# douban/dpark

Measured on NVIDIA H100. Metric: shuffled rows/sec (reduceByKey end-to-end), higher is better.
Workload: dtype int64

## Files before the change

__graft_entry__.py:

```python
import os
import subprocess
import sys

ROOT = os.path.dirname(os.path.abspath(__file__))
if ROOT not in sys.path:
    sys.path.insert(0, ROOT)


def build():
    subprocess.check_call(["make", "-s", "-j8", "-C", os.path.join(ROOT, "dpark_b200", "csrc")])
    subprocess.check_call(["make", "-s", "-C", os.path.join(ROOT, "oracle"), "all"])
    from oracle import build_reference
    if os.path.exists(os.path.join(build_reference.REF, "dpark", "portable_hash.pyx")):
        subprocess.call(["make", "-s", "-C", os.path.join(ROOT, "oracle"), "ref", "REF=" + build_reference.REF])
        subprocess.call([sys.executable, os.path.join(ROOT, "oracle", "build_reference.py")])
    subprocess.check_call(
        ["nvcc", "-gencode", "arch=compute_90a,code=sm_90a", "-O2", "-std=c++17", "-Xcompiler", "-fPIC",
         "-shared", "-I" + os.path.join(ROOT, "include"), "-I" + os.path.join(ROOT, "dpark_b200", "csrc"),
         os.path.join(ROOT, "tests", "hostcheck.cu"), os.path.join(ROOT, "dpark_b200", "csrc", "dpk_core.o"),
         "-o", os.path.join(ROOT, "tests", "_hostcheck.so")])
    import dpark_b200
    from dpark_b200 import _native
    _native.lib()


def smoke():
    import numpy as np
    import torch
    from dpark_b200 import _native as nv
    from dpark_b200 import shuffle
    from oracle import oracle as orc

    assert torch.cuda.is_available(), "smoke() needs cuda:0"
    torch.cuda.set_device(0)
    rng = np.random.default_rng(0)
    n, P, M = 200000, 8, 4
    k = rng.integers(-5000, 5000, n, dtype=np.int64)
    v = rng.integers(0, 1 << 16, n, dtype=np.int64)
    ks, vs = np.array_split(k, M), np.array_split(v, M)
    before = nv.launch_count()
    res = shuffle.reduce_by_key([torch.from_numpy(x).cuda() for x in ks],
                                [torch.from_numpy(x).cuda() for x in vs], P, "sum")
    torch.cuda.synchronize()
    assert nv.launch_count() > before, "no CUDA kernels were launched"
    want = orc.reduce_by_key(ks, vs, P, "sum")
    for p, gk, gv in res:
        gk, gv = gk.cpu().numpy(), gv.cpu().numpy()
        wk, wv = want[p]
        o1, o2 = np.argsort(gk), np.argsort(wk)
        assert np.array_equal(gk[o1], wk[o2]) and np.array_equal(gv[o1], wv[o2]), "partition %d differs" % p
    print("smoke ok: reduceByKey over %d rows, %d partitions, %d kernel launches, matches oracle"
          % (n, P, nv.launch_count() - before))


if __name__ == "__main__":
    build()
    if len(sys.argv) > 1 and sys.argv[1] == "smoke":
        smoke()
```

dpark_b200/csrc/dpk_common.cuh:

```cuda
#pragma once
#include <cuda_runtime.h>
#include <stdint.h>
#include <stdio.h>
#include <stdarg.h>
#include <string.h>
#include <math.h>

#include "dpark_b200.h"

#define DPK_HD __host__ __device__ __forceinline__

namespace dpk {

extern thread_local char g_err[512];
int fail(int code, const char *fmt, ...);
#define DPK_CUDA_TRY(expr)                                                        \
    do {                                                                          \
        cudaError_t _e = (expr);                                                  \
        if (_e != cudaSuccess)                                                    \
            return dpk::fail(DPK_ERR_CUDA, "%s failed: %s (%s:%d)", #expr,        \
                             cudaGetErrorString(_e), __FILE__, __LINE__);         \
    } while (0)
#define DPK_LAUNCH_CHECK() DPK_CUDA_TRY(cudaGetLastError())

// ... 110 lines not shown
struct PartFn {
    int32_t P;
    int32_t mode;
    uint64_t magic;
    int32_t shift;
    int32_t nthr;
    const int64_t *thresholds;
    int32_t sub_bits;
    const int64_t *row_hash;

    DPK_HD int32_t nbuckets() const { return P << sub_bits; }
    DPK_HD int32_t bucket(int64_t h) const {
        if (mode == 4) return (int32_t)(((uint64_t)h >> shift) & (uint64_t)(P - 1));
        if (mode == 5) return P == 1 ? 0 : (int32_t)((mixed(h) >> shift) & (uint32_t)(P - 1));
        int32_t p = (*this)(h);
        if (sub_bits == 0) return p;
        return (p << sub_bits) | (int32_t)(mixed(h) >> (32 - sub_bits));
    }
    static DPK_HD uint32_t mixed(int64_t h) {
        uint32_t x = (uint32_t)(uint64_t)h * 0x9E3779B1u + (uint32_t)((uint64_t)h >> 32) * 0x85EBCA77u;
        x ^= x >> 16; x *= 0x21F0AAADu;
        x ^= x >> 15; x *= 0x735A2D97u;
        x ^= x >> 15;
        return x;
    }

    DPK_HD int32_t operator()(int64_t h) const {
        if (mode == 1) return (int32_t)((uint64_t)h & (uint64_t)(P - 1));
        if (mode == 2) {
            uint64_t a = h < 0 ? 0ull - (uint64_t)h : (uint64_t)h;
#ifdef __CUDA_ARCH__
            uint64_t q = __umul64hi(magic, a);
#else
            uint64_t q = (uint64_t)(((unsigned __int128)magic * a) >> 64);
#endif
            uint64_t t = ((a - q) >> 1) + q;
            q = t >> shift;
            uint32_t r = (uint32_t)(a - q * (uint64_t)P);
            return h < 0 ? (r ? P - (int32_t)r : 0) : (int32_t)r;
        }
        if (mode == 3) {
            int32_t lo = 0, hi = nthr;
            while (lo < hi) {
                int32_t mid = (lo + hi) >> 1;
                if (h < thresholds[mid]) hi = mid; else lo = mid + 1;
            }
            return lo;
        }
        return 0;
    }
};
int make_partfn(int32_t P, const int64_t *thresholds, int32_t nthr, int32_t sub_bits, PartFn *out);

int64_t seg_multisplit_ws_bytes(int64_t n, int32_t F1, int32_t S2, int32_t nsrc);
int seg_multisplit(const void *keys, int key_kind, const void *vals, int32_t val_bytes, int64_t n,
                   const PartFn &fine, int32_t F1, int32_t nsrc, const int64_t *seg_start,
                   const int64_t *seg_rows, void *out_keys, void *out_vals, int64_t *fine_off, void *ws,
                   int64_t ws_bytes, cudaStream_t st, bool stable = false);

DPK_HD uint64_t mix64(uint64_t x) {
    x ^= x >> 33; x *= 0xff51afd7ed558ccdull; x ^= x >> 33; x *= 0xc4ceb9fe1a85ec53ull;
    return x ^ (x >> 33);
}
DPK_HD uint32_t slot_hash32(uint64_t kb) {
    uint32_t x = (uint32_t)kb * 0xCC9E2D51u + (uint32_t)(kb >> 32) * 0x1B873593u + 0x7F4A7C15u;
    x ^= x >> 16; x *= 0x85EBCA6Bu;
    x ^= x >> 13; x *= 0xC2B2AE35u;
    x ^= x >> 16;
    return x;
}

constexpr int AG_MAX_SB2 = 10;
DPK_HD int choose_sb2(int64_t n, int32_t F, int target_rows) {
    int sb2 = 0;
    while (sb2 < AG_MAX_SB2 && n / ((int64_t)F << sb2) > target_rows) sb2++;
    return sb2;
}
DPK_HD PartFn fine_partfn(const PartFn &first, int sb2) {
    PartFn fine = first;
    fine.mode = 5; fine.P = 1 << sb2; fine.shift = 32 - first.sub_bits - sb2; fine.sub_bits = 0;
    return fine;
}

constexpr int TK_BYTES = 16;
__host__ __device__ __forceinline__ bool tok_ws(uint8_t c) { return c == 0x20 || (c >= 0x09 && c <= 0x0d) || (c >= 0x1c && c <= 0x1f); }

__host__ __device__ __forceinline__ uint32_t tok_starts16(const uint8_t *__restrict__ data, int64_t n, int64_t i0, bool *hi) {
    uint8_t c[TK_BYTES];
    if (i0 + TK_BYTES <= n && (((uintptr_t)(data + i0)) & 15u) == 0) {
        const uint4 q = *reinterpret_cast<const uint4 *>(data + i0);
        const uint32_t w[4] = {q.x, q.y, q.z, q.w};
#pragma unroll
        for (int j = 0; j < TK_BYTES; j++) c[j] = (uint8_t)(w[j >> 2] >> ((j & 3) * 8));
    } else {
#pragma unroll
        for (int j = 0; j < TK_BYTES; j++) c[j] = i0 + j < n ? data[i0 + j] : (uint8_t)0x20;
    }
    bool prev_ws = i0 == 0 ? true : tok_ws(data[i0 - 1]);
    uint32_t m = 0;
    bool h = false;
#pragma unroll
    for (int j = 0; j < TK_BYTES; j++) {
        const bool ws = tok_ws(c[j]);
        h |= c[j] >= 0x80;
        if (!ws && prev_ws) m |= 1u << j;
        prev_ws = ws;
    }
    *hi = h;
    return m;
}


}
```

dpark_b200/csrc/dpk_partition.cu:

```cuda
#include "dpk_common.cuh"

namespace dpk {

constexpr int PT_THREADS = 256;
constexpr int PT_WARPS = PT_THREADS / 32;
constexpr int PT_ITEMS = 16;
constexpr int PT_TILE = PT_THREADS * PT_ITEMS;
constexpr int PT_COUNT_PRIV = 1024;

struct NoVal {};

int g_count_mode = 1;
int g_scatter_items = 16;
int g_scatter_bulk = 1;
int g_scatter_threads = 512;
int g_scatter_seg_wide = 1;
int g_scatter_wide_from = 512;
int g_scatter_ptr_bulk = 1;
int g_scatter_ptr_threads = 1024;

struct SegTab {
    const int64_t *cbeg, *cend;
    const int32_t *ctotal;
    int32_t *chunk_counts;
    const int64_t *chunk_off;
    const uint64_t *key_ptrs, *val_ptrs;
    int unordered;
};

struct Plan {
    int32_t T;
    int64_t L;
    SegTab seg;
    const char *label_count = nullptr, *label_scatter = nullptr;
};

static Plan make_plan(int64_t n) {
    Plan pl;
    pl.seg = SegTab{nullptr, nullptr, nullptr, nullptr, nullptr, nullptr, nullptr, 0};
    int64_t tiles = (n + PT_TILE - 1) / PT_TILE;
    if (tiles < 1) tiles = 1;
    int64_t maxT = (int64_t)sm_count() * 8;
    pl.T = (int32_t)(tiles < maxT ? tiles : maxT);
    pl.L = tiles;
    return pl;
}

static inline int64_t align_up(int64_t x, int64_t a) { return (x + a - 1) / a * a; }

static int64_t ws_counts_bytes(int32_t P) { return align_up((int64_t)P * sm_count() * 8 * 4, 256); }
static int64_t ws_total_bytes(int32_t P) {
    return ws_counts_bytes(P) + align_up((int64_t)P * 8, 256) + align_up((int64_t)(P + 1) * 8, 256);
}

template <typename KeyT, int PRE>
__device__ __forceinline__ int64_t key_hash(KeyT k, const PartFn &f) {
    if constexpr (PRE == 1) return (int64_t)k;
    else if constexpr (PRE == 2) return __ldg(&f.row_hash[(int64_t)k]);
    else return KeyHash<KeyT>::of(k);
}

__device__ __forceinline__ unsigned warp_peers(int id, int nbits) {
    unsigned peers = 0xffffffffu;
#pragma unroll
    for (int b = 0; b < 13; b++) {
        if (b < nbits) {
            const unsigned set = __ballot_sync(0xffffffffu, (id >> b) & 1);
            peers &= ((id >> b) & 1) ? set : ~set;
        }
    }
    return peers;
}

template <int NW = PT_WARPS>
__device__ __forceinline__ int block_excl_scan(int v, int *s_warp, int *total) {
    const int lane = threadIdx.x & 31, warp = threadIdx.x >> 5;
    int inc = v;
#pragma unroll
    for (int d = 1; d < 32; d <<= 1) {
        int t = __shfl_up_sync(0xffffffffu, inc, d);
        if (lane >= d) inc += t;
    }
    if (lane == 31) s_warp[warp] = inc;
    __syncthreads();
    int base = 0, tot = 0;
#pragma unroll
    for (int w = 0; w < NW; w++) {
        int t = s_warp[w];
        if (w < warp) base += t;
        tot += t;
    }
    __syncthreads();
    *total = tot;
    return base + inc - v;
}

template <typename KeyT, int PRE>
__global__ void __launch_bounds__(PT_THREADS)
k_part_count(const KeyT *__restrict__ keys, int64_t n, int64_t L, PartFn f,
             int32_t *__restrict__ tile_counts, int32_t T, SegTab seg, int count_mode) {
    extern __shared__ int32_t s_cnt[];
    const int P = f.nbuckets();
    if (seg.cbeg != nullptr && (int)blockIdx.x >= *seg.ctotal) return;
    const bool priv = P <= PT_COUNT_PRIV;
    const int nhist = priv ? PT_WARPS * P : P;
    for (int p = threadIdx.x; p < nhist; p += PT_THREADS) s_cnt[p] = 0;
    __syncthreads();
    const int64_t beg = seg.cbeg ? seg.cbeg[blockIdx.x] : ((int64_t)blockIdx.x * L / T) * PT_TILE;
    const int64_t end = seg.cbeg ? seg.cend[blockIdx.x] : min(n, ((int64_t)(blockIdx.x + 1) * L / T) * PT_TILE);
    const int lane = threadIdx.x & 31;
    int32_t *wh = s_cnt + (priv ? (threadIdx.x >> 5) * P : 0);
    constexpr int U = 8;
    int64_t i0 = beg;
    if (count_mode == 1) {
        for (; i0 + (int64_t)PT_THREADS * U <= end; i0 += (int64_t)PT_THREADS * U) {
            KeyT k[U];
#pragma unroll
            for (int u = 0; u < U; u++) k[u] = keys[i0 + (int64_t)u * PT_THREADS + threadIdx.x];
#pragma unroll
            for (int u = 0; u < U; u++) atomicAdd(&wh[f.bucket(key_hash<KeyT, PRE>(k[u], f))], 1);
        }
    }
    for (; i0 < end; i0 += (int64_t)PT_THREADS * U) {
        KeyT k[U];
        bool ok[U];
#pragma unroll
        for (int u = 0; u < U; u++) {
            int64_t i = i0 + (int64_t)u * PT_THREADS + threadIdx.x;
            ok[u] = i < end;
            k[u] = ok[u] ? keys[i] : KeyT(0);
        }
// ... 359 lines not shown
                const int p = bucket_of<FMODE>(f, key_hash<KeyT, PRE>(k[j], f));
                pr[j] = ((uint32_t)p << 16) | atomicAdd(&cnt[p], 1u);
            }
        } else {
            const int left = (int)(end - tile) - warp * (32 * ITEMS) - lane;
#pragma unroll
            for (int j = 0; j < ITEMS; j++) {
                pr[j] = 0xffffffffu;
                if (j * 32 < left) {
                    const int p = bucket_of<FMODE>(f, key_hash<KeyT, PRE>(k[j], f));
                    pr[j] = ((uint32_t)p << 16) | atomicAdd(&cnt[p], 1u);
                }
            }
        }
        asm volatile("cp.async.bulk.wait_group.read 0;" ::: "memory");
        __syncthreads();

        {
            const int b = threadIdx.x * E;
            int sum = 0;
            for (int i = b; i < min(b + E, P); i++) sum += (int)cnt[i];
            int tot;
            int run = block_excl_scan<NW>(sum, s_warp, &tot);
            for (int i = b; i < min(b + E, P); i++) {
                const int64_t g = s_gpos[i];
                const uint32_t gk = (uint32_t)(((uintptr_t)(out_keys + g)) / sizeof(KeyT));
                const int basek = run + i * (AK - 1);
                s_sk[i] = basek + (int)((gk - (uint32_t)basek) & (uint32_t)(AK - 1));
                if constexpr (HAS_VAL) {
                    const uint32_t gv = (uint32_t)(((uintptr_t)(out_vals + (ptrs ? g + s_vd[i] : g))) / sizeof(ValT));
                    const int basev = run + i * (AV - 1);
                    s_sv[i] = basev + (int)((gv - (uint32_t)basev) & (uint32_t)(AV - 1));
                }
                run += (int)cnt[i];
            }
        }
        __syncthreads();

#pragma unroll
        for (int j = 0; j < ITEMS; j++) {
            const int p = (int)(pr[j] >> 16), r = (int)(pr[j] & 0xffffu);
            if (p != 0xffff) {
                s_key[s_sk[p] + r] = k[j];
                if constexpr (HAS_VAL) s_val[s_sv[p] + r] = v[j];
            }
        }
        if (tile + TILE < end) load_tile(tile + TILE);
        asm volatile("fence.proxy.async.shared::cta;" ::: "memory");
        __syncthreads();

        if constexpr (HAS_VAL) {
            for (int q0 = 0; q0 < 2 * P; q0 += NT) {
                const int q = q0 + (int)threadIdx.x;
                const int p = q >> 1;
                const bool on = q < 2 * P;
                const int c = on ? (int)cnt[p] : 0;
                const int64_t g = on ? s_gpos[p] : 0;
                if (c) {
                    if (q & 1) flush_run<ValT>(out_vals, ptrs ? g + s_vd[p] : g, s_val, val_addr, s_sv[p], c);
                    else flush_run<KeyT>(out_keys, g, s_key, key_addr, s_sk[p], c);
                }
                __syncwarp();
                if (c && !(q & 1)) {
                    s_gpos[p] = g + c;
                    cnt[p] = 0;
                }
            }
        } else {
            for (int p = threadIdx.x; p < P; p += NT) {
                const int c = (int)cnt[p];
                if (c) {
                    const int64_t g = s_gpos[p];
                    flush_run<KeyT>(out_keys, g, s_key, key_addr, s_sk[p], c);
                    s_gpos[p] = g + c;
                    cnt[p] = 0;
                }
            }
        }
        asm volatile("cp.async.bulk.commit_group;" ::: "memory");
    }
    asm volatile("cp.async.bulk.wait_group 0;" ::: "memory");
}

template <typename KeyT, int PRE>
static int launch_count(const void *keys, int64_t n, const Plan &pl, const PartFn &f,
                        int32_t *tile_counts, cudaStream_t st) {
    size_t sh = (size_t)f.nbuckets() * sizeof(int32_t) * (f.nbuckets() <= PT_COUNT_PRIV ? PT_WARPS : 1);
    DPK_LAUNCH(pl.label_count ? pl.label_count : (pl.seg.cbeg ? "seg_count" : "part_count"), st, k_part_count<KeyT, PRE><<<pl.T, PT_THREADS, sh, st>>>((const KeyT *)keys, n, pl.L, f, tile_counts, pl.T, pl.seg, g_count_mode));
    return DPK_OK;
}

static int dispatch_count(const void *keys, int key_kind, int64_t n, const Plan &pl, const PartFn &f,
                          int32_t *tile_counts, cudaStream_t st) {
    if (key_kind >= DPK_K_UNORDERED) key_kind -= DPK_K_UNORDERED;
    switch (key_kind) {
    case -1: return launch_count<int64_t, true>(keys, n, pl, f, tile_counts, st);
    case DPK_K_I64: return launch_count<int64_t, false>(keys, n, pl, f, tile_counts, st);
    case DPK_K_I32: return launch_count<int32_t, false>(keys, n, pl, f, tile_counts, st);
    case DPK_K_F64: return launch_count<double, false>(keys, n, pl, f, tile_counts, st);
    case DPK_K_U64: return launch_count<uint64_t, false>(keys, n, pl, f, tile_counts, st);
    case DPK_K_F32: return launch_count<float, false>(keys, n, pl, f, tile_counts, st);
    case DPK_K_ROWID:
        if (!f.row_hash) return fail(DPK_ERR_INVALID, "DPK_K_ROWID needs key_aux (the per-row hash column)");
        return launch_count<int64_t, 2>(keys, n, pl, f, tile_counts, st);
    }
    return fail(DPK_ERR_UNSUPPORTED, "key kind %d is unhashable by portable_hash", key_kind);
}

template <typename KeyT, typename ValT, int PRE, int ITEMS>
static int launch_scatter_items(const void *keys, const void *vals, int64_t n, const Plan &pl, const PartFn &f,
                                const int32_t *tile_off, const int64_t *bucket_base, void *out_keys,
                                void *out_vals, cudaStream_t st) {
    constexpr int vb = std::is_same<ValT, NoVal>::value ? 0 : (int)sizeof(ValT);
    ScatterSmem lay = scatter_smem((int)sizeof(KeyT), vb, f.nbuckets(), pl.seg.key_ptrs != nullptr, PT_THREADS * ITEMS);
    auto kern = k_part_scatter<KeyT, ValT, PRE, ITEMS>;
    if (lay.total > 227 * 1024)
        return fail(DPK_ERR_UNSUPPORTED, "%d buckets need %lld B of shared memory", f.nbuckets(), (long long)lay.total);
    DPK_CUDA_TRY(cudaFuncSetAttribute(kern, cudaFuncAttributeMaxDynamicSharedMemorySize, (int)lay.total));
    DPK_LAUNCH(pl.label_scatter ? pl.label_scatter : (pl.seg.cbeg ? "seg_scatter" : "part_scatter"), st,
               kern<<<pl.T, PT_THREADS, (size_t)lay.total, st>>>((const KeyT *)keys, (const ValT *)vals, n, pl.L, f,
                                                                tile_off, pl.T, bucket_base, (KeyT *)out_keys,
                                                                (ValT *)out_vals, lay, pl.seg));
    return DPK_OK;
}

template <typename KeyT, typename ValT, int PRE>
static int launch_scatter_bulk(const void *keys, const void *vals, int64_t n, const Plan &pl, const PartFn &f,
                               const int32_t *tile_off, const int64_t *bucket_base, void *out_keys,
                               void *out_vals, cudaStream_t st) {
    constexpr int vb = std::is_same<ValT, NoVal>::value ? 0 : (int)sizeof(ValT);
    int nt = g_scatter_threads;
    if (nt == 512 && pl.seg.cbeg != nullptr && g_scatter_seg_wide) nt = 1024;
    if (nt == 512 && g_scatter_seg_wide && sizeof(KeyT) <= 4 && (vb == 0 || vb <= 4)) nt = 1024;
    if (nt == 512 && g_scatter_wide_from > 0 && f.nbuckets() >= g_scatter_wide_from) nt = 1024;
    const bool ptr_mode = pl.seg.key_ptrs != nullptr;
    if (ptr_mode && nt == 512 && g_scatter_ptr_threads == 1024) nt = 1024;
    if (nt == 1024 && bulk_smem((int)sizeof(KeyT), vb, f.nbuckets(), 8192, ptr_mode).total > 220 * 1024) nt = 512;
    BulkSmem lay = bulk_smem((int)sizeof(KeyT), vb, f.nbuckets(), nt == 1024 ? 8192 : PT_TILE, ptr_mode);
    const int fmode = f.mode == 5 ? 2 : ((f.mode == 0 || f.mode == 1) ? 1 : 0);
    if (ptr_mode) {
        auto kp = nt == 1024 ? (fmode == 1 ? k_part_scatter_bulk<KeyT, ValT, PRE, 1024, 1, true> : k_part_scatter_bulk<KeyT, ValT, PRE, 1024, 0, true>)
                             : (fmode == 1 ? k_part_scatter_bulk<KeyT, ValT, PRE, 512, 1, true> : k_part_scatter_bulk<KeyT, ValT, PRE, 512, 0, true>);
        if (nt != 512 && nt != 1024) return fail(DPK_ERR_UNSUPPORTED, "pointer mode needs 512- or 1024-thread CTAs");
        DPK_CUDA_TRY(cudaFuncSetAttribute(kp, cudaFuncAttributeMaxDynamicSharedMemorySize, (int)lay.total));
        DPK_LAUNCH(pl.label_scatter ? pl.label_scatter : "part_scatter", st,
                   kp<<<pl.T, nt, (size_t)lay.total, st>>>((const KeyT *)keys, (const ValT *)vals, n, pl.L, f, tile_off, pl.T,
                                                          bucket_base, (KeyT *)out_keys, (ValT *)out_vals, lay, pl.seg));
        return DPK_OK;
    }
    auto kern = nt == 1024 ? (fmode == 2 ? k_part_scatter_bulk<KeyT, ValT, PRE, 1024, 2> :
                              fmode == 1 ? k_part_scatter_bulk<KeyT, ValT, PRE, 1024, 1> : k_part_scatter_bulk<KeyT, ValT, PRE, 1024, 0>)
              : nt == 512 ? (fmode == 2 ? k_part_scatter_bulk<KeyT, ValT, PRE, 512, 2> :
                             fmode == 1 ? k_part_scatter_bulk<KeyT, ValT, PRE, 512, 1> : k_part_scatter_bulk<KeyT, ValT, PRE, 512, 0>)
                          : k_part_scatter_bulk<KeyT, ValT, PRE, 256, 0>;
    DPK_CUDA_TRY(cudaFuncSetAttribute(kern, cudaFuncAttributeMaxDynamicSharedMemorySize, (int)lay.total));
    DPK_LAUNCH(pl.label_scatter ? pl.label_scatter : (pl.seg.cbeg ? "seg_scatter" : "part_scatter"), st,
               kern<<<pl.T, nt, (size_t)lay.total, st>>>((const KeyT *)keys, (const ValT *)vals, n, pl.L, f,
                                                                tile_off, pl.T, bucket_base, (KeyT *)out_keys,
                                                                (ValT *)out_vals, lay, pl.seg));
    return DPK_OK;
}

template <typename KeyT, typename ValT, int PRE>
static int launch_scatter(const void *keys, const void *vals, int64_t n, const Plan &pl_in, const PartFn &f,
                          const int32_t *tile_off, const int64_t *bucket_base, void *out_keys,
                          void *out_vals, cudaStream_t st) {
    Plan pl = pl_in;
    if (pl.seg.unordered == 2) {
        constexpr int vb = std::is_same<ValT, NoVal>::value ? 0 : (int)sizeof(ValT);
        if (bulk_smem((int)sizeof(KeyT), vb, f.nbuckets(), PT_TILE, pl.seg.key_ptrs != nullptr).total <= 110 * 1024)
            return launch_scatter_bulk<KeyT, ValT, PRE>(keys, vals, n, pl, f, tile_off, bucket_base, out_keys, out_vals, st);
        pl.seg.unordered = (f.nbuckets() % 2 == 0) ? 1 : 0;
    }
    if (g_scatter_items == 8)
        return launch_scatter_items<KeyT, ValT, PRE, 8>(keys, vals, n, pl, f, tile_off, bucket_base, out_keys, out_vals, st);
    return launch_scatter_items<KeyT, ValT, PRE, 16>(keys, vals, n, pl, f, tile_off, bucket_base, out_keys, out_vals, st);
}

template <typename KeyT, int PRE>
static int dispatch_val(const void *keys, const void *vals, int32_t val_bytes, int64_t n, const Plan &pl,
                        const PartFn &f, const int32_t *tile_off, const int64_t *bucket_base,
                        void *out_keys, void *out_vals, cudaStream_t st) {
    if (vals == nullptr || val_bytes == 0)
        return launch_scatter<KeyT, NoVal, PRE>(keys, nullptr, n, pl, f, tile_off, bucket_base, out_keys, nullptr, st);
    if (val_bytes == 8)
        return launch_scatter<KeyT, int64_t, PRE>(keys, vals, n, pl, f, tile_off, bucket_base, out_keys, out_vals, st);
    if (val_bytes == 4)
        return launch_scatter<KeyT, int32_t, PRE>(keys, vals, n, pl, f, tile_off, bucket_base, out_keys, out_vals, st);
    return fail(DPK_ERR_UNSUPPORTED, "val_bytes must be 0, 4 or 8, got %d", val_bytes);
}

static int dispatch_scatter(const void *keys, int key_kind, const void *vals, int32_t val_bytes, int64_t n,
                            const Plan &pl_in, const PartFn &f, const int32_t *tile_off,
                            const int64_t *bucket_base, void *out_keys, void *out_vals, cudaStream_t st) {
    Plan pl = pl_in;
    if (key_kind >= DPK_K_UNORDERED) {
        key_kind -= DPK_K_UNORDERED;
        if (f.nbuckets() % 2 == 0) pl.seg.unordered = 1;
        if (g_scatter_bulk && (pl.seg.key_ptrs == nullptr || g_scatter_ptr_bulk)) pl.seg.unordered = 2;
    } else if (pl.seg.unordered && g_scatter_bulk && pl.seg.key_ptrs == nullptr) {
        pl.seg.unordered = 2;
    }
    switch (key_kind) {
    case -1: return dispatch_val<int64_t, true>(keys, vals, val_bytes, n, pl, f, tile_off, bucket_base, out_keys, out_vals, st);
    case DPK_K_I64: return dispatch_val<int64_t, false>(keys, vals, val_bytes, n, pl, f, tile_off, bucket_base, out_keys, out_vals, st);
    case DPK_K_I32: return dispatch_val<int32_t, false>(keys, vals, val_bytes, n, pl, f, tile_off, bucket_base, out_keys, out_vals, st);
    case DPK_K_F64: return dispatch_val<double, false>(keys, vals, val_bytes, n, pl, f, tile_off, bucket_base, out_keys, out_vals, st);
    case DPK_K_U64: return dispatch_val<uint64_t, false>(keys, vals, val_bytes, n, pl, f, tile_off, bucket_base, out_keys, out_vals, st);
    case DPK_K_F32: return dispatch_val<float, false>(keys, vals, val_bytes, n, pl, f, tile_off, bucket_base, out_keys, out_vals, st);
    case DPK_K_ROWID:
        if (!f.row_hash) return fail(DPK_ERR_INVALID, "DPK_K_ROWID needs key_aux (the per-row hash column)");
        return dispatch_val<int64_t, 2>(keys, vals, val_bytes, n, pl, f, tile_off, bucket_base, out_keys, out_vals, st);
    }
    return fail(DPK_ERR_UNSUPPORTED, "key kind %d is unhashable by portable_hash", key_kind);
}

static int check_common(const void *keys, int64_t n, int32_t P, int32_t sub_bits, void *ws, int64_t ws_bytes) {
    if (n < 0 || n >= ((int64_t)1 << 31)) return fail(DPK_ERR_INVALID, "n=%lld out of range [0, 2^31)", (long long)n);
    if (P < 1 || sub_bits < 0 || sub_bits > 12 || ((int64_t)P << sub_bits) > DPK_MAX_PARTITIONS)
        return fail(DPK_ERR_UNSUPPORTED, "P=%d (x 2^%d sub-buckets) out of range [1, %d]", P, sub_bits, DPK_MAX_PARTITIONS);
    P <<= sub_bits;
    if (n > 0 && !keys) return fail(DPK_ERR_INVALID, "keys is NULL");
// ... 68 lines not shown
        int t = s_tot[p];
        s_tot[p] = run;
        run += t;
    }
    __syncthreads();
    const int64_t base = brow_off[b];
    for (int p = threadIdx.x; p < S2; p += PT_THREADS) {
        int64_t pos = base + s_tot[p];
        fine_off[(int64_t)b * S2 + p] = pos;
        for (int64_t c = c0; c < c1; c++) {
            chunk_off[c * S2 + p] = pos;
            pos += chunk_counts[c * S2 + p];
        }
    }
    if (b == F1 - 1 && threadIdx.x == 0) fine_off[(int64_t)F1 * S2] = brow_off[F1];
}

int64_t seg_multisplit_ws_bytes(int64_t n, int32_t F1, int32_t S2, int32_t nsrc) {
    const int64_t maxc = seg_max_chunks(n, F1, nsrc);
    return align_up((int64_t)(F1 + 1) * 8, 256) * 2 + 256 + align_up(maxc * 8, 256) * 2 +
           align_up(maxc * S2 * 4, 256) + align_up(maxc * S2 * 8, 256);
}

int seg_multisplit(const void *keys, int key_kind, const void *vals, int32_t val_bytes, int64_t n,
                   const PartFn &fine, int32_t F1, int32_t nsrc, const int64_t *seg_start,
                   const int64_t *seg_rows, void *out_keys, void *out_vals, int64_t *fine_off, void *ws,
                   int64_t ws_bytes, cudaStream_t st, bool stable) {
    const int32_t S2 = fine.nbuckets();
    if (ws_bytes < seg_multisplit_ws_bytes(n, F1, S2, nsrc)) return fail(DPK_ERR_WORKSPACE, "segmented multisplit workspace too small");
    const int64_t maxc = seg_max_chunks(n, F1, nsrc);
    char *w = (char *)ws;
    int64_t *brow_off = (int64_t *)w; w += align_up((int64_t)(F1 + 1) * 8, 256);
    int64_t *cfirst = (int64_t *)w; w += align_up((int64_t)(F1 + 1) * 8, 256);
    int32_t *ctotal = (int32_t *)w; w += 256;
    int64_t *cbeg = (int64_t *)w; w += align_up(maxc * 8, 256);
    int64_t *cend = (int64_t *)w; w += align_up(maxc * 8, 256);
    int32_t *chunk_counts = (int32_t *)w; w += align_up(maxc * S2 * 4, 256);
    int64_t *chunk_off = (int64_t *)w;
    DPK_LAUNCH("seg_plan", st, k_seg_plan<<<1, PT_THREADS, 0, st>>>(seg_start, seg_rows, nsrc, F1, brow_off, cfirst, cbeg, cend, ctotal));
    Plan pl;
    pl.T = (int32_t)maxc;
    pl.L = 0;
    pl.seg = SegTab{cbeg, cend, ctotal, chunk_counts, chunk_off, nullptr, nullptr, (S2 % 2 == 0) ? 1 : (g_scatter_bulk ? 2 : 0)};
    if (stable) {
        pl.seg.unordered = 0;
        pl.label_count = "radix_count";
        pl.label_scatter = "radix_scatter";
    }
    int rc = DPK_OK;
    if (n > 0) {
        rc = dispatch_count(keys, key_kind, n, pl, fine, nullptr, st);
        if (rc) return rc;
    }
    DPK_LAUNCH("seg_scan", st, k_seg_scan<<<F1, PT_THREADS, (size_t)S2 * 4, st>>>(chunk_counts, cfirst, brow_off, F1, S2, chunk_off, fine_off));
    if (n > 0) rc = dispatch_scatter(keys, key_kind, vals, val_bytes, n, pl, fine, nullptr, nullptr, out_keys, out_vals, st);
    return rc;
}

}

using namespace dpk;

extern "C" {

int64_t dpk_partition_workspace_bytes(int64_t n, int32_t nbuckets) {
    (void)n;
    if (nbuckets < 1) nbuckets = 1;
    return ws_total_bytes(nbuckets);
}

int dpk_partition_count(const void *keys, int key_kind, const int64_t *key_aux, int64_t n, int32_t P,
                        const int64_t *thresholds, int32_t nthr, int32_t sub_bits, int64_t *out_counts,
                        void *ws, int64_t ws_bytes, dpk_stream_t stream) {
    int rc = check_common(keys, n, P, sub_bits, ws, ws_bytes);
    if (rc) return rc;
    if (!out_counts) return fail(DPK_ERR_INVALID, "out_counts is NULL");
    PartFn f;
    rc = make_partfn(P, thresholds, nthr, sub_bits, &f);
    if (rc) return rc;
    f.row_hash = key_aux;
    const int32_t F = f.nbuckets();
    cudaStream_t st = (cudaStream_t)stream;
    int32_t *tile_counts = (int32_t *)ws;
    Plan pl = make_plan(n);
    if (n == 0) {
        DPK_CUDA_TRY(cudaMemsetAsync(tile_counts, 0, (size_t)F * pl.T * 4, st));
    } else {
        rc = dispatch_count(keys, key_kind, n, pl, f, tile_counts, st);
        if (rc) return rc;
    }
    DPK_LAUNCH("part_scan", st, k_part_scan<<<F, PT_THREADS, 0, st>>>(tile_counts, pl.T, out_counts));
    return DPK_OK;
}

int dpk_partition_scatter(const void *keys, int key_kind, const int64_t *key_aux, const void *vals,
                          int32_t val_bytes, int64_t n, int32_t P, const int64_t *thresholds, int32_t nthr,
                          int32_t sub_bits,
                          const int64_t *bucket_base, void *out_keys, void *out_vals, void *ws,
                          int64_t ws_bytes, dpk_stream_t stream) {
    int rc = check_common(keys, n, P, sub_bits, ws, ws_bytes);
    if (rc) return rc;
    if (n == 0) return DPK_OK;
    if (!bucket_base || !out_keys) return fail(DPK_ERR_INVALID, "NULL pointer");
    PartFn f;
    rc = make_partfn(P, thresholds, nthr, sub_bits, &f);
    if (rc) return rc;
    f.row_hash = key_aux;
    Plan pl = make_plan(n);
    return dispatch_scatter(keys, key_kind, vals, val_bytes, n, pl, f, (const int32_t *)ws, bucket_base,
                            out_keys, out_vals, (cudaStream_t)stream);
}

int dpk_partition(const void *keys, int key_kind, const int64_t *key_aux, const void *vals, int32_t val_bytes,
                  int64_t n, int32_t P, const int64_t *thresholds, int32_t nthr, int32_t sub_bits, void *out_keys, void *out_vals,
                  int64_t *out_offsets, void *ws, int64_t ws_bytes, dpk_stream_t stream) {
    int rc = check_common(keys, n, P, sub_bits, ws, ws_bytes);
    if (rc) return rc;
    if (!out_offsets) return fail(DPK_ERR_INVALID, "out_offsets is NULL");
    const int32_t F = P << sub_bits;
    int64_t *totals = (int64_t *)((char *)ws + ws_counts_bytes(F));
    rc = dpk_partition_count(keys, key_kind, key_aux, n, P, thresholds, nthr, sub_bits, totals, ws, ws_bytes, stream);
    if (rc) return rc;
    cudaStream_t st = (cudaStream_t)stream;
    DPK_LAUNCH("part_offsets", st, k_part_offsets<<<1, PT_THREADS, 0, st>>>(totals, F, out_offsets));
    return dpk_partition_scatter(keys, key_kind, key_aux, vals, val_bytes, n, P, thresholds, nthr, sub_bits, out_offsets,
                                 out_keys, out_vals, ws, ws_bytes, stream);
}

int dpk_partition_scatter_ptrs(const void *keys, int key_kind, const int64_t *key_aux, const void *vals,
                               int32_t val_bytes, int64_t n, int32_t P, const int64_t *thresholds, int32_t nthr,
                               int32_t sub_bits, const uint64_t *key_dst_ptrs, const uint64_t *val_dst_ptrs,
                               void *ws, int64_t ws_bytes, dpk_stream_t stream) {
    int rc = check_common(keys, n, P, sub_bits, ws, ws_bytes);
    if (rc) return rc;
    if (n == 0) return DPK_OK;
    if (!key_dst_ptrs || (vals && val_bytes && !val_dst_ptrs)) return fail(DPK_ERR_INVALID, "NULL pointer table");
    PartFn f;
    rc = make_partfn(P, thresholds, nthr, sub_bits, &f);
    if (rc) return rc;
    f.row_hash = key_aux;
    Plan pl = make_plan(n);
    pl.seg.key_ptrs = key_dst_ptrs;
    pl.seg.val_ptrs = val_dst_ptrs;
    return dispatch_scatter(keys, key_kind, vals, val_bytes, n, pl, f, (const int32_t *)ws, nullptr, nullptr, nullptr,
                            (cudaStream_t)stream);
}

__global__ void __launch_bounds__(PT_THREADS)
k_seg_starts(const int64_t *__restrict__ seg_rows, int32_t nsrc, int32_t F, int64_t *__restrict__ seg_start) {
    __shared__ long long s_part[PT_THREADS];
    __shared__ long long s_carry;
    const int E = (F + PT_THREADS - 1) / PT_THREADS;
    const int b0 = threadIdx.x * E, b1 = min(b0 + E, F);
    if (threadIdx.x == 0) s_carry = 0;
    __syncthreads();
    for (int s = 0; s < nsrc; s++) {
        long long mine = 0;
        for (int b = b0; b < b1; b++) mine += seg_rows[(int64_t)s * F + b];
        s_part[threadIdx.x] = mine;
        __syncthreads();
        long long base = s_carry, tot = 0;
        for (int t = 0; t < PT_THREADS; t++) {
            if (t < (int)threadIdx.x) base += s_part[t];
            tot += s_part[t];
        }
        for (int b = b0; b < b1; b++) {
            seg_start[(int64_t)s * F + b] = base;
            base += seg_rows[(int64_t)s * F + b];
        }
        __syncthreads();
        if (threadIdx.x == 0) s_carry += tot;
        __syncthreads();
    }
}

int64_t dpk_radix_pass_seg_workspace_bytes(int64_t n, int32_t nbuckets, int32_t nsrc, int32_t bits) {
    if (n < 0) n = 0;
    if (nbuckets < 1) nbuckets = 1;
    if (nsrc < 1) nsrc = 1;
    return align_up((int64_t)nbuckets * nsrc * 8, 256) + seg_multisplit_ws_bytes(n, nbuckets, 1 << bits, nsrc);
}

int dpk_radix_pass_seg(const int64_t *keys, const void *vals, int32_t val_bytes, int64_t n, int32_t shift, int32_t bits,
                       int32_t nbuckets, int32_t nsrc, const int64_t *seg_rows, int64_t *out_keys, void *out_vals,
                       int64_t *out_fine_off, void *ws, int64_t ws_bytes, dpk_stream_t stream) {
    if (bits < 1 || bits > 10 || shift < 0 || shift > 63) return fail(DPK_ERR_INVALID, "bad radix digit shift=%d bits=%d", shift, bits);
    if (n < 0 || n >= ((int64_t)1 << 31)) return fail(DPK_ERR_INVALID, "n=%lld out of range [0, 2^31)", (long long)n);
    if (nbuckets < 1 || nsrc < 1 || !seg_rows || !out_fine_off || !ws) return fail(DPK_ERR_INVALID, "bad segment description");
    if (n > 0 && (!keys || !out_keys)) return fail(DPK_ERR_INVALID, "NULL pointer");
    if (ws_bytes < dpk_radix_pass_seg_workspace_bytes(n, nbuckets, nsrc, bits)) return fail(DPK_ERR_WORKSPACE, "workspace too small");
    cudaStream_t st = (cudaStream_t)stream;
    int64_t *seg_start = (int64_t *)ws;
    void *ws2 = (char *)ws + align_up((int64_t)nbuckets * nsrc * 8, 256);
    DPK_LAUNCH("seg_starts", st, k_seg_starts<<<1, PT_THREADS, 0, st>>>(seg_rows, nsrc, nbuckets, seg_start));
    PartFn f;
    f.P = 1 << bits; f.mode = 4; f.magic = 0; f.shift = shift; f.nthr = 0; f.thresholds = nullptr; f.sub_bits = 0;
    f.row_hash = nullptr;
    return seg_multisplit(keys, -1, vals, val_bytes, n, f, nbuckets, nsrc, seg_start, seg_rows, out_keys, out_vals,
                          out_fine_off, ws2, ws_bytes - align_up((int64_t)nbuckets * nsrc * 8, 256), st, true);
}

int dpk_radix_pass(const int64_t *keys, const void *vals, int32_t val_bytes, int64_t n, int32_t shift,
                   int32_t bits, int64_t *out_keys, void *out_vals, void *ws, int64_t ws_bytes,
                   dpk_stream_t stream) {
    if (bits < 1 || bits > 12 || shift < 0 || shift > 63)
        return fail(DPK_ERR_INVALID, "bad radix digit shift=%d bits=%d", shift, bits);
    const int32_t F = 1 << bits;
    int rc = check_common(keys, n, F, 0, ws, ws_bytes);
    if (rc) return rc;
    if (n == 0) return DPK_OK;
    if (!out_keys) return fail(DPK_ERR_INVALID, "NULL pointer");
    PartFn f;
    f.P = F; f.mode = 4; f.magic = 0; f.shift = shift; f.nthr = 0; f.thresholds = nullptr; f.sub_bits = 0;
    f.row_hash = nullptr;
    cudaStream_t st = (cudaStream_t)stream;
    int32_t *tile_counts = (int32_t *)ws;
    int64_t *totals = (int64_t *)((char *)ws + ws_counts_bytes(F));
    int64_t *offsets = (int64_t *)((char *)totals + align_up((int64_t)F * 8, 256));
    Plan pl = make_plan(n);
    pl.label_count = "radix_count";
    pl.label_scatter = "radix_scatter";
    rc = dispatch_count(keys, -1, n, pl, f, tile_counts, st);
    if (rc) return rc;
    DPK_LAUNCH("part_scan", st, k_part_scan<<<F, PT_THREADS, 0, st>>>(tile_counts, pl.T, totals));
// ... 6 lines not shown
```

Baseline: 15.42 billion.

## Add 2-CTA cluster scatter kernel sharing staging buffers via distributed shared memory

Adds a thread-block-cluster variant of the bulk partition scatter, used for unordered keys with many buckets. The two CTAs in a cluster combine their per-bucket counts through distributed shared memory and write rows into a shared staging buffer split across both CTAs, so each bulk flush covers longer contiguous runs. The grid size is also reworked to be a multiple of the number of active clusters. The aim is fewer, larger bulk copies to global memory when buckets are small. The cost is two cluster barriers per tile and remote shared-memory stores.

```diff
diff --git a/__graft_entry__.py b/__graft_entry__.py
--- a/__graft_entry__.py
+++ b/__graft_entry__.py
@@ -19,6 +19,10 @@
          "-shared", "-I" + os.path.join(ROOT, "include"), "-I" + os.path.join(ROOT, "dpark_b200", "csrc"),
          os.path.join(ROOT, "tests", "hostcheck.cu"), os.path.join(ROOT, "dpark_b200", "csrc", "dpk_core.o"),
          "-o", os.path.join(ROOT, "tests", "_hostcheck.so")])
+    subprocess.check_call(
+        ["nvcc", "-gencode", "arch=compute_90a,code=sm_90a", "-O2", "-std=c++17", "-Xcompiler", "-fPIC",
+         "-shared", "-I" + os.path.join(ROOT, "include"), "-I" + os.path.join(ROOT, "dpark_b200", "csrc"),
+         os.path.join(ROOT, "tests", "hostcheck_cluster.cu"), "-o", os.path.join(ROOT, "tests", "_hostcheck_cluster.so")])
     import dpark_b200
     from dpark_b200 import _native
     _native.lib()
diff --git a/dpark_b200/csrc/dpk_common.cuh b/dpark_b200/csrc/dpk_common.cuh
--- a/dpark_b200/csrc/dpk_common.cuh
+++ b/dpark_b200/csrc/dpk_common.cuh
@@ -216,6 +216,28 @@
     return fine;
 }
 
+DPK_HD int cluster_run_start(int run, int p, uint32_t dst, int A) {
+    const int base = run + p * (A - 1);
+    return base + (int)((dst - (uint32_t)base) & (uint32_t)(A - 1));
+}
+DPK_HD int cluster_slice_slots(int tile, int P, int C, int A) {
+    const int s = tile + (P * (A - 1) + C - 1) / C;
+    return (s + A - 1) / A * A;
+}
+DPK_HD int cluster_owner(int L, int S, int C) {
+    int o = 0;
+    for (int q = 1; q < C; q++) o += L >= q * S;
+    return o;
+}
+DPK_HD int cluster_piece(int start, int cnt, int o, int S, int *s0, int *off) {
+    const int lo = start > o * S ? start : o * S;
+    const int hi = start + cnt < (o + 1) * S ? start + cnt : (o + 1) * S;
+    if (hi <= lo) return 0;
+    *s0 = lo - o * S;
+    *off = lo - start;
+    return hi - lo;
+}
+
 constexpr int TK_BYTES = 16;
 __host__ __device__ __forceinline__ bool tok_ws(uint8_t c) { return c == 0x20 || (c >= 0x09 && c <= 0x0d) || (c >= 0x1c && c <= 0x1f); }
 
diff --git a/dpark_b200/csrc/dpk_partition.cu b/dpark_b200/csrc/dpk_partition.cu
--- a/dpark_b200/csrc/dpk_partition.cu
+++ b/dpark_b200/csrc/dpk_partition.cu
@@ -28,14 +28,21 @@
     int unordered;
 };
 
+static inline int64_t align_up(int64_t x, int64_t a) { return (x + a - 1) / a * a; }
+
 struct Plan {
     int32_t T;
     int64_t L;
     SegTab seg;
     const char *label_count = nullptr, *label_scatter = nullptr;
+    int32_t cluster = 1;
 };
 
-static Plan make_plan(int64_t n) {
+constexpr int SCATTER_CLUSTER = 2;
+constexpr int CLUSTER_FROM = 512;
+static int active_clusters();
+
+static Plan make_plan(int64_t n, int32_t F = 0, bool unordered = false) {
     Plan pl;
     pl.seg = SegTab{nullptr, nullptr, nullptr, nullptr, nullptr, nullptr, nullptr, 0};
     int64_t tiles = (n + PT_TILE - 1) / PT_TILE;
@@ -43,10 +50,24 @@
     int64_t maxT = (int64_t)sm_count() * 8;
     pl.T = (int32_t)(tiles < maxT ? tiles : maxT);
     pl.L = tiles;
+    constexpr int C = SCATTER_CLUSTER;
+    if (unordered && g_scatter_bulk && F >= CLUSTER_FROM && active_clusters() > 0) {
+        pl.cluster = C;
+        const int64_t slots = (int64_t)active_clusters() * C;
+        if (tiles < slots) {
+            pl.T = (int32_t)align_up(tiles, C);
+        } else {
+            int64_t best = 0, best_cost = 0;
+            for (int64_t w = 1; w <= 8; w++) {
+                const int64_t per = (tiles + w * slots - 1) / (w * slots);
+                const int64_t cost = w * ((per * PT_TILE + 8191) / 8192);
+                if (best == 0 || cost <= best_cost) { best = w; best_cost = cost; }
+            }
+            pl.T = (int32_t)(best * slots);
+        }
+    }
     return pl;
 }
-
-static inline int64_t align_up(int64_t x, int64_t a) { return (x + a - 1) / a * a; }
 
 static int64_t ws_counts_bytes(int32_t P) { return align_up((int64_t)P * sm_count() * 8 * 4, 256); }
 static int64_t ws_total_bytes(int32_t P) {
@@ -572,6 +593,220 @@
     asm volatile("cp.async.bulk.wait_group 0;" ::: "memory");
 }
 
+struct ClusterSmem {
+    int64_t key_off, val_off, gpos_off, cnt_off, rk_off, rv_off, sk_off, sv_off, tot_off, total;
+    int32_t key_slots, val_slots;
+};
+static ClusterSmem cluster_smem(int kb, int vb, int32_t P, int C, int tile) {
+    ClusterSmem s;
+    int64_t o = 0;
+    s.key_slots = cluster_slice_slots(tile, P, C, 16 / kb);
+    s.val_slots = vb ? cluster_slice_slots(tile, P, C, 16 / vb) : 0;
+    s.key_off = o; o += align_up((int64_t)s.key_slots * kb, 128);
+    s.val_off = o; o += align_up((int64_t)s.val_slots * vb, 128);
+    s.gpos_off = o; o += align_up((int64_t)P * 8, 16);
+    s.cnt_off = o; o += align_up((int64_t)P * 4 * 2, 16);
+    s.rk_off = o; o += align_up((int64_t)P * 4, 16);
+    s.rv_off = o; o += align_up((int64_t)P * 4, 16);
+    s.sk_off = o; o += align_up((int64_t)P * 4, 16);
+    s.sv_off = o; o += align_up((int64_t)P * 4, 16);
+    s.tot_off = o; o += align_up((int64_t)P * 4, 16);
+    s.total = o;
+    return s;
+}
+
+__device__ __forceinline__ uint32_t cluster_map(uint32_t addr, uint32_t rank) {
+    uint32_t r;
+    asm volatile("mapa.shared::cluster.u32 %0, %1, %2;" : "=r"(r) : "r"(addr), "r"(rank));
+    return r;
+}
+__device__ __forceinline__ void cluster_barrier() {
+    asm volatile("barrier.cluster.arrive.release.aligned;\n\tbarrier.cluster.wait.acquire.aligned;" ::: "memory");
+}
+template <typename T>
+__device__ __forceinline__ void st_cluster(uint32_t addr, T v) {
+    if constexpr (sizeof(T) == 8) {
+        uint64_t b;
+        memcpy(&b, &v, 8);
+        asm volatile("st.shared::cluster.b64 [%0], %1;" ::"r"(addr), "l"(b) : "memory");
+    } else {
+        uint32_t b;
+        memcpy(&b, &v, 4);
+        asm volatile("st.shared::cluster.b32 [%0], %1;" ::"r"(addr), "r"(b) : "memory");
+    }
+}
+
+template <typename KeyT, typename ValT, int PRE, int FMODE, int C>
+__global__ void __launch_bounds__(1024, 1)
+k_part_scatter_cluster(const KeyT *__restrict__ keys, const ValT *__restrict__ vals, int64_t n, int64_t L,
+                       PartFn f, const int32_t *__restrict__ tile_off, int32_t T,
+                       const int64_t *__restrict__ bucket_base, KeyT *__restrict__ out_keys,
+                       ValT *__restrict__ out_vals, ClusterSmem lay) {
+    constexpr bool HAS_VAL = !std::is_same<ValT, NoVal>::value;
+    constexpr int NT = 1024, ITEMS = 8, TILE = NT * ITEMS, NW = NT / 32;
+    constexpr int AK = 16 / (int)sizeof(KeyT);
+    constexpr int AV = HAS_VAL ? 16 / (int)sizeof(typename std::conditional<HAS_VAL, ValT, int64_t>::type) : 1;
+    extern __shared__ __align__(128) unsigned char smem_cl[];
+    __shared__ int s_warp[NW];
+    KeyT *s_key = reinterpret_cast<KeyT *>(smem_cl + lay.key_off);
+    ValT *s_val = reinterpret_cast<ValT *>(smem_cl + lay.val_off);
+    int64_t *s_gpos = reinterpret_cast<int64_t *>(smem_cl + lay.gpos_off);
+    uint32_t *s_cnt = reinterpret_cast<uint32_t *>(smem_cl + lay.cnt_off);
+    int32_t *s_rk = reinterpret_cast<int32_t *>(smem_cl + lay.rk_off);
+    int32_t *s_rv = reinterpret_cast<int32_t *>(smem_cl + lay.rv_off);
+    int32_t *s_sk = reinterpret_cast<int32_t *>(smem_cl + lay.sk_off);
+    int32_t *s_sv = reinterpret_cast<int32_t *>(smem_cl + lay.sv_off);
+    int32_t *s_tot = reinterpret_cast<int32_t *>(smem_cl + lay.tot_off);
+    const uint32_t key_addr = (uint32_t)__cvta_generic_to_shared(s_key);
+    const uint32_t val_addr = (uint32_t)__cvta_generic_to_shared(s_val);
+    const int SK = lay.key_slots, SV = lay.val_slots;
+
+    const int P = f.nbuckets();
+    const int lane = threadIdx.x & 31, warp = threadIdx.x >> 5;
+#define CRANK ((int)(blockIdx.x % C))
+    const int c0 = (int)blockIdx.x - CRANK;
+    const int64_t beg = ((int64_t)blockIdx.x * L / T) * PT_TILE;
+    const int len = (int)max((int64_t)0, min(n, ((int64_t)(blockIdx.x + 1) * L / T) * PT_TILE) - beg);
+    int iters = 0;
+#pragma unroll
+    for (int o = 0; o < C; o++) {
+        const int64_t b = ((int64_t)(c0 + o) * L / T) * PT_TILE, e = min(n, ((int64_t)(c0 + o + 1) * L / T) * PT_TILE);
+        if (e > b) iters = max(iters, (int)((e - b + TILE - 1) / TILE));
+    }
+    for (int p = threadIdx.x; p < P; p += NT) s_gpos[p] = bucket_base[p] + (int64_t)tile_off[(int64_t)p * T + c0];
+    for (int p = threadIdx.x; p < 2 * P; p += NT) s_cnt[p] = 0;
+    const int E = (P + NT - 1) / NT;
+
+    KeyT k[ITEMS];
+    ValT v[ITEMS];
+    const int64_t first = beg + warp * (32 * ITEMS) + lane;
+    const int left0 = len - warp * (32 * ITEMS) - lane;
+    auto load_tile = [&](int t) {
+        const KeyT *kp = keys + first + (int64_t)t * TILE;
+        const int left = left0 - t * TILE;
+#pragma unroll
+        for (int j = 0; j < ITEMS; j++) k[j] = j * 32 < left ? kp[j * 32] : KeyT(0);
+        if constexpr (HAS_VAL) {
+            const ValT *vp = vals + first + (int64_t)t * TILE;
+#pragma unroll
+            for (int j = 0; j < ITEMS; j++)
+                if (j * 32 < left) v[j] = vp[j * 32];
+        }
+    };
+    if (len > 0) load_tile(0);
+    __syncthreads();
+
+    int par = 0;
+    for (int it = 0; it < iters; it++, par ^= 1) {
+        uint32_t *cnt = s_cnt + par * P;
+        uint32_t pr[ITEMS];
+        {
+            const int left = left0 - it * TILE;
+#pragma unroll
+            for (int j = 0; j < ITEMS; j++) {
+                pr[j] = 0xffffffffu;
+                if (j * 32 < left) {
+                    const int p = bucket_of<FMODE>(f, key_hash<KeyT, PRE>(k[j], f));
+                    pr[j] = ((uint32_t)p << 16) | atomicAdd(&cnt[p], 1u);
+                }
+            }
+        }
+        asm volatile("cp.async.bulk.wait_group.read 0;" ::: "memory");
+        cluster_barrier();
+
+        {
+            const int b = threadIdx.x * E;
+            const uint32_t caddr = key_addr + (uint32_t)(lay.cnt_off - lay.key_off) + (uint32_t)(par * P) * 4u;
+            int sum = 0;
+            for (int i = b; i < min(b + E, P); i++) {
+                int tot = 0, mine = 0;
+#pragma unroll
+                for (int o = 0; o < C; o++) {
+                    uint32_t c;
+                    asm volatile("ld.shared::cluster.u32 %0, [%1];" : "=r"(c) : "r"(cluster_map(caddr + (uint32_t)i * 4u, (uint32_t)o)) : "memory");
+                    if (o < CRANK) mine += (int)c;
+                    tot += (int)c;
+                }
+                s_tot[i] = tot;
+                s_sk[i] = mine;
+                sum += tot;
+            }
+            int total;
+            int run = block_excl_scan<NW>(sum, s_warp, &total);
+            for (int i = b; i < min(b + E, P); i++) {
+                const int64_t g = s_gpos[i];
+                const int rk = cluster_run_start(run, i, (uint32_t)((uintptr_t)out_keys / sizeof(KeyT)) + (uint32_t)g, AK);
+                const int mine = s_sk[i];
+                s_rk[i] = rk;
+                s_sk[i] = rk + mine;
+                if constexpr (HAS_VAL) {
+                    const int rv = cluster_run_start(run, i, (uint32_t)((uintptr_t)out_vals / sizeof(ValT)) + (uint32_t)g, AV);
+                    s_rv[i] = rv;
+                    s_sv[i] = rv + mine;
+                }
+                run += s_tot[i];
+            }
+        }
+        __syncthreads();
+
+#pragma unroll
+        for (int j = 0; j < ITEMS; j++) {
+            const int p = (int)(pr[j] >> 16), r = (int)(pr[j] & 0xffffu);
+            if (p != 0xffff) {
+                const int lk = s_sk[p] + r, ok = cluster_owner(lk, SK, C);
+                st_cluster<KeyT>(cluster_map(key_addr + (uint32_t)(lk - ok * SK) * (uint32_t)sizeof(KeyT), (uint32_t)ok), k[j]);
+                if constexpr (HAS_VAL) {
+                    const int lv = s_sv[p] + r, ov = cluster_owner(lv, SV, C);
+                    st_cluster<ValT>(cluster_map(val_addr + (uint32_t)(lv - ov * SV) * (uint32_t)sizeof(ValT), (uint32_t)ov), v[j]);
+                }
+            }
+        }
+        if ((it + 1) * TILE < len) load_tile(it + 1);
+        asm volatile("fence.proxy.async.shared::cluster;" ::: "memory");
+        cluster_barrier();
+
+        if constexpr (HAS_VAL) {
+            for (int q0 = 0; q0 < 2 * P; q0 += NT) {
+                const int q = q0 + (int)threadIdx.x;
+                const int p = q >> 1;
+                const bool on = q < 2 * P;
+                const int c = on ? s_tot[p] : 0;
+                const int64_t g = on ? s_gpos[p] : 0;
+                if (c) {
+                    int s0, off;
+                    if (q & 1) {
+                        const int m = cluster_piece(s_rv[p], c, CRANK, SV, &s0, &off);
+                        if (m) flush_run<ValT>(out_vals, g + off, s_val, val_addr, s0, m);
+                    } else {
+                        const int m = cluster_piece(s_rk[p], c, CRANK, SK, &s0, &off);
+                        if (m) flush_run<KeyT>(out_keys, g + off, s_key, key_addr, s0, m);
+                    }
+                }
+                __syncwarp();
+                if (c && !(q & 1)) {
+                    s_gpos[p] = g + c;
+                    cnt[p] = 0;
+                }
+            }
+        } else {
+            for (int p = threadIdx.x; p < P; p += NT) {
+                const int c = s_tot[p];
+                if (c) {
+                    const int64_t g = s_gpos[p];
+                    int s0, off;
+                    const int m = cluster_piece(s_rk[p], c, CRANK, SK, &s0, &off);
+                    if (m) flush_run<KeyT>(out_keys, g + off, s_key, key_addr, s0, m);
+                    s_gpos[p] = g + c;
+                    cnt[p] = 0;
+                }
+            }
+        }
+        asm volatile("cp.async.bulk.commit_group;" ::: "memory");
+    }
+    asm volatile("cp.async.bulk.wait_group 0;" ::: "memory");
+#undef CRANK
+}
+
 template <typename KeyT, int PRE>
 static int launch_count(const void *keys, int64_t n, const Plan &pl, const PartFn &f,
                         int32_t *tile_counts, cudaStream_t st) {
@@ -614,6 +849,56 @@
     return DPK_OK;
 }
 
+template <int C>
+static cudaLaunchConfig_t cluster_config(dim3 grid, size_t smem, cudaStream_t st, cudaLaunchAttribute *attr) {
+    cudaLaunchConfig_t cfg = {};
+    cfg.gridDim = grid;
+    cfg.blockDim = dim3(1024);
+    cfg.dynamicSmemBytes = smem;
+    cfg.stream = st;
+    attr->id = cudaLaunchAttributeClusterDimension;
+    attr->val.clusterDim.x = C;
+    attr->val.clusterDim.y = 1;
+    attr->val.clusterDim.z = 1;
+    cfg.attrs = attr;
+    cfg.numAttrs = 1;
+    return cfg;
+}
+
+static int active_clusters() {
+    static int cached = -1;
+    if (cached >= 0) return cached;
+    constexpr int C = SCATTER_CLUSTER;
+    auto kern = k_part_scatter_cluster<int64_t, int64_t, 0, 1, C>;
+    const ClusterSmem lay = cluster_smem(8, 8, CLUSTER_FROM, C, 8192);
+    cudaLaunchAttribute attr;
+    cudaLaunchConfig_t cfg = cluster_config<C>(dim3(C * 64), (size_t)lay.total, 0, &attr);
+    int active = 0;
+    if (cudaFuncSetAttribute(kern, cudaFuncAttributeMaxDynamicSharedMemorySize, (int)lay.total) != cudaSuccess ||
+        cudaOccupancyMaxActiveClusters(&active, kern, &cfg) != cudaSuccess) {
+        cudaGetLastError();
+        active = 0;
+    }
+    cached = active;
+    return cached;
+}
+
+template <typename KeyT, typename ValT, int PRE, int C>
+static int launch_scatter_cluster(const void *keys, const void *vals, int64_t n, const Plan &pl, const PartFn &f,
+                                  const int32_t *tile_off, const int64_t *bucket_base, void *out_keys,
+                                  void *out_vals, cudaStream_t st) {
+    constexpr int vb = std::is_same<ValT, NoVal>::value ? 0 : (int)sizeof(ValT);
+    const ClusterSmem lay = cluster_smem((int)sizeof(KeyT), vb, f.nbuckets(), C, 8192);
+    auto kern = (f.mode == 0 || f.mode == 1) ? k_part_scatter_cluster<KeyT, ValT, PRE, 1, C> : k_part_scatter_cluster<KeyT, ValT, PRE, 0, C>;
+    DPK_CUDA_TRY(cudaFuncSetAttribute(kern, cudaFuncAttributeMaxDynamicSharedMemorySize, (int)lay.total));
+    cudaLaunchAttribute attr;
+    cudaLaunchConfig_t cfg = cluster_config<C>(dim3(pl.T), (size_t)lay.total, st, &attr);
+    DPK_LAUNCH(pl.label_scatter ? pl.label_scatter : "part_scatter", st,
+               DPK_CUDA_TRY(cudaLaunchKernelEx(&cfg, kern, (const KeyT *)keys, (const ValT *)vals, n, pl.L, f, tile_off, pl.T,
+                                               bucket_base, (KeyT *)out_keys, (ValT *)out_vals, lay)));
+    return DPK_OK;
+}
+
 template <typename KeyT, typename ValT, int PRE>
 static int launch_scatter_bulk(const void *keys, const void *vals, int64_t n, const Plan &pl, const PartFn &f,
                                const int32_t *tile_off, const int64_t *bucket_base, void *out_keys,
@@ -628,6 +913,9 @@
     if (nt == 1024 && bulk_smem((int)sizeof(KeyT), vb, f.nbuckets(), 8192, ptr_mode).total > 220 * 1024) nt = 512;
     BulkSmem lay = bulk_smem((int)sizeof(KeyT), vb, f.nbuckets(), nt == 1024 ? 8192 : PT_TILE, ptr_mode);
     const int fmode = f.mode == 5 ? 2 : ((f.mode == 0 || f.mode == 1) ? 1 : 0);
+    if (nt == 1024 && pl.cluster > 1 && pl.seg.cbeg == nullptr && !ptr_mode)
+        return launch_scatter_cluster<KeyT, ValT, PRE, SCATTER_CLUSTER>(keys, vals, n, pl, f, tile_off, bucket_base, out_keys,
+                                                                         out_vals, st);
     if (ptr_mode) {
         auto kp = nt == 1024 ? (fmode == 1 ? k_part_scatter_bulk<KeyT, ValT, PRE, 1024, 1, true> : k_part_scatter_bulk<KeyT, ValT, PRE, 1024, 0, true>)
                              : (fmode == 1 ? k_part_scatter_bulk<KeyT, ValT, PRE, 512, 1, true> : k_part_scatter_bulk<KeyT, ValT, PRE, 512, 0, true>);
@@ -862,7 +1150,7 @@
     const int32_t F = f.nbuckets();
     cudaStream_t st = (cudaStream_t)stream;
     int32_t *tile_counts = (int32_t *)ws;
-    Plan pl = make_plan(n);
+    Plan pl = make_plan(n, F, key_kind >= DPK_K_UNORDERED);
     if (n == 0) {
         DPK_CUDA_TRY(cudaMemsetAsync(tile_counts, 0, (size_t)F * pl.T * 4, st));
     } else {
@@ -886,7 +1174,7 @@
     rc = make_partfn(P, thresholds, nthr, sub_bits, &f);
     if (rc) return rc;
     f.row_hash = key_aux;
-    Plan pl = make_plan(n);
+    Plan pl = make_plan(n, f.nbuckets(), key_kind >= DPK_K_UNORDERED);
     return dispatch_scatter(keys, key_kind, vals, val_bytes, n, pl, f, (const int32_t *)ws, bucket_base,
                             out_keys, out_vals, (cudaStream_t)stream);
 }
@@ -919,7 +1207,7 @@
     rc = make_partfn(P, thresholds, nthr, sub_bits, &f);
     if (rc) return rc;
     f.row_hash = key_aux;
-    Plan pl = make_plan(n);
+    Plan pl = make_plan(n, f.nbuckets(), key_kind >= DPK_K_UNORDERED);
     pl.seg.key_ptrs = key_dst_ptrs;
     pl.seg.val_ptrs = val_dst_ptrs;
     return dispatch_scatter(keys, key_kind, vals, val_bytes, n, pl, f, (const int32_t *)ws, nullptr, nullptr, nullptr,
```

After: 16.27 billion, median of 6. 5.5% higher.
